# INK-USC/RE-Net

Hardware: AMD Instinct MI355X
Metric: RGCN+GRU encoder triples/s at bs=1024 n_hidden=200 (full training step, both directions) (higher is better)
Workload: dtype f32; 1 GPU; ICEWS18-shaped synthetic stream (seed 999), n_hidden=200, seq_len=10, batch=1024 per GPU, dropout=0.50, fwd+bwd both directions + clip + Adam; parallelism=dp1, global_batch=1024, nodes=99312, edges=288792

## Files before the change

re-net_amd/csrc/common.h:

```cpp
#pragma once
#include <hip/hip_runtime.h>
#include <stdint.h>
#include <stdlib.h>
#include <string.h>
#include "../../include/renet_hip.h"

#define RENET_LAUNCH(...)                         \
    do {                                          \
        (void)hipGetLastError();                  \
        hipLaunchKernelGGL(__VA_ARGS__);          \
    } while (0)

#define RENET_LAUNCH_CHECK()                      \
    do {                                          \
        hipError_t e__ = hipGetLastError();       \
        if (e__ != hipSuccess) return (int)e__;   \
    } while (0)

static inline bool renet_env_flag(const char* name, bool dflt) {
    const char* e = getenv(name);
    return (e && e[0] == '0') ? false : (e && e[0] == '1') ? true : dflt;
}
static inline int renet_env_int(const char* name, int dflt, int lo, int hi) {
    const char* e = getenv(name);
    const int v = e ? atoi(e) : dflt;
    return (v < lo || v > hi) ? dflt : v;
}
static inline bool renet_env_is(const char* name, const char* value) {
    const char* e = getenv(name);
    return e && strcmp(e, value) == 0;
}

static inline int renet_gemm_tile_order() {
    static const int v = renet_env_flag("RENET_GEMM_TILE_ORDER", true) ? renet_env_int("RENET_GEMM_PANEL_W", 8, 1, 64) : 0;
    return v;
}

static inline bool renet_dim_ok(int D) { return D == 100 || D == 200 || D == 300 || D == 400; }

__device__ __forceinline__ uint64_t renet_mix64(uint64_t x) {
    x += 0x9E3779B97F4A7C15ull;
    x = (x ^ (x >> 30)) * 0xBF58476D1CE4E5B9ull;
    x = (x ^ (x >> 27)) * 0x94D049BB133111EBull;
    return x ^ (x >> 31);
}

struct DropCfg {
    uint32_t thresh;
    float scale;
    uint64_t seed;
};

static inline DropCfg make_drop(float p, uint64_t seed) {
    DropCfg d;
    if (p <= 0.f) { d.thresh = 0; d.scale = 1.f; }
    else { d.thresh = (uint32_t)(p * 65536.f + 0.5f); d.scale = 1.f / (1.f - p); }
    d.seed = seed;
// ... 35 lines not shown
```

re-net_amd/csrc/gemm_bf16s.hip:

```cpp
#include "gemm_tiles.h"

namespace {

constexpr int P3_LOADERS = 4;
constexpr int P3_THREADS = 64 * (4 + P3_LOADERS);

struct Bf16sArgs {
    const __bf16* A;
    const __bf16* B;
    int lda, ldb;
    SplitArgs out;
};

constexpr int B1_SUB = 2;
constexpr int B1_BK = 32 * B1_SUB;
constexpr int B1_STAGE = 2 * B1_SUB * 8192;
constexpr int B1_SLOTS = 3;
constexpr size_t B1_LDS = (size_t)B1_STAGE * B1_SLOTS;
constexpr size_t B1_LDS_TALL = (size_t)B1_SUB * (256 * 64 + 8192) * B1_SLOTS;

template <bool A_TR, bool B_TR, bool TALL>
__global__ __launch_bounds__(TALL ? 768 : P3_THREADS) void gemm_bf16s_kernel(Bf16sArgs pa) {
    constexpr int TBM = TALL ? 256 : 128;
    constexpr int MW = TALL ? 8 : 4;
// ... 141 lines not shown
#pragma unroll
            for (int slab = 0; slab < 2; ++slab)
#pragma unroll
                for (int t = 0; t < 2; ++t) {
                    const char* ia = st + sb * AIMG;
                    const char* ib = st + B1_SUB * AIMG + sb * 8192;
                    if constexpr (!A_TR) fa[sb][slab][t] = *reinterpret_cast<const bf16x8*>(ia + offA[t][slab]);
                    else fa[sb][slab][t] = frag_tr(ia, offA[t], slab);
                    if constexpr (!B_TR) fb[sb][slab][t] = *reinterpret_cast<const bf16x8*>(ib + offB[t][slab]);
                    else fb[sb][slab][t] = frag_tr(ib, offB[t], slab);
                }
#pragma unroll
        for (int sb = 0; sb < B1_SUB; ++sb)
#pragma unroll
            for (int slab = 0; slab < 2; ++slab)
#pragma unroll
                for (int i = 0; i < 2; ++i)
#pragma unroll
                    for (int j = 0; j < 2; ++j)
                        acc[i][j] = __builtin_amdgcn_mfma_f32_32x32x16_bf16(fa[sb][slab][i], fb[sb][slab][j], acc[i][j], 0, 0, 0);
        asm volatile("s_waitcnt lgkmcnt(0)" ::: "memory");
        __builtin_amdgcn_s_barrier();
    }
    store_tile(g, m0, n0, z, wm, wn, lane, acc);
}

__global__ __launch_bounds__(256) void pack_bf16_kernel(const float* __restrict__ X, int R, int C, int ldx, int Rp,
                                                        int Cp, __bf16* __restrict__ P) {
    const size_t total = (size_t)Rp * Cp / 4;
    for (size_t i = (size_t)blockIdx.x * blockDim.x + threadIdx.x; i < total; i += (size_t)gridDim.x * blockDim.x) {
        const int row = (int)(i / (Cp / 4)), c = (int)(i % (Cp / 4)) * 4;
        float4 v = make_float4(0.f, 0.f, 0.f, 0.f);
        if (row < R) {
            const float* x = X + (size_t)row * ldx + c;
            if (c + 3 < C && ((ldx & 3) == 0) && ((reinterpret_cast<uintptr_t>(X) & 15) == 0)) {
                v = *reinterpret_cast<const float4*>(x);
            } else {
                if (c < C) v.x = x[0];
                if (c + 1 < C) v.y = x[1];
                if (c + 2 < C) v.z = x[2];
                if (c + 3 < C) v.w = x[3];
            }
        }
        const bf16x2 lo = __builtin_convertvector(f32x2{v.x, v.y}, bf16x2);
        const bf16x2 hi = __builtin_convertvector(f32x2{v.z, v.w}, bf16x2);
        *reinterpret_cast<uint2*>(P + (size_t)row * Cp + c) = pack4(lo, hi);
    }
// ... 52 lines not shown
}

int renet_gemm_bf16s(int a_tr, int b_tr, int M, int N, int K, float alpha, const void* Ap, int lda, const void* Bp,
                     int ldb, float beta, float* C, int ldc, const float* bias, int split_k, float* workspace,
                     size_t workspace_bytes, void* stream) {
    if (M < 0 || N < 0 || K < 1 || ldc < N || !Ap || !Bp) return RENET_ERR_BADARG;
    if (M == 0 || N == 0) return RENET_OK;
    const int Mp = (M + 255) & ~255, Np = (N + 255) & ~255, Kp = (K + 255) & ~255;
    if (lda < (a_tr ? Mp : Kp) || ldb < (b_tr ? Np : Kp) || (lda & 7) || (ldb & 7)) return RENET_ERR_BADARG;
    if (split_k < 1) split_k = 1;
    const int st_total = (K + B1_BK - 1) / B1_BK;
    if (split_k > st_total) split_k = max(st_total, 1);
    if (split_k > 1 && workspace_bytes < renet_gemm_workspace(M, N, split_k)) return RENET_ERR_WORKSPACE;
    Bf16sArgs pa;
    pa.A = (const __bf16*)Ap; pa.B = (const __bf16*)Bp;
    pa.lda = lda; pa.ldb = ldb;
    SplitArgs& g = pa.out;
    g.A = nullptr; g.B = nullptr; g.C = C; g.bias = bias; g.M = M; g.N = N; g.K = K;
    g.lda = 0; g.ldb = 0; g.ldc = ldc; g.alpha = alpha; g.beta = beta;
    g.split_k = split_k;
    g.k_tiles_per_split = max(1, (st_total + split_k - 1) / split_k);
    g.partial = workspace;
    g.xcd_order = renet_gemm_tile_order();
    hipStream_t st = (hipStream_t)stream;
    const int nbx = (N + BN - 1) / BN;
    const bool tall = (size_t)nbx * (Mp / 256) * split_k >= 256;
    dim3 grid(nbx, tall ? Mp / 256 : (M + BM - 1) / BM, split_k);
    int e;
    if (tall) {
        if (!a_tr && !b_tr) e = launch_bf16s<false, false, true>(pa, grid, st);
        else if (!a_tr && b_tr) e = launch_bf16s<false, true, true>(pa, grid, st);
        else if (a_tr && !b_tr) e = launch_bf16s<true, false, true>(pa, grid, st);
        else e = launch_bf16s<true, true, true>(pa, grid, st);
    } else {
        if (!a_tr && !b_tr) e = launch_bf16s<false, false, false>(pa, grid, st);
        else if (!a_tr && b_tr) e = launch_bf16s<false, true, false>(pa, grid, st);
        else if (a_tr && !b_tr) e = launch_bf16s<true, false, false>(pa, grid, st);
        else e = launch_bf16s<true, true, false>(pa, grid, st);
    }
    if (e != RENET_OK) return e;
    if (split_k > 1) return renet_split_reduce(workspace, split_k, M, N, alpha, beta, bias, C, ldc, st);
    return RENET_OK;
}

}
```

re-net_amd/csrc/gemm_h3.hip:

```cpp
#include <type_traits>
#include "gemm_tiles.h"
#include "gemm_skinny.h"

namespace {

typedef _Float16 f16x8 __attribute__((ext_vector_type(8)));
typedef _Float16 f16x2 __attribute__((ext_vector_type(2)));

struct H3Args {
    SplitArgs g;
    const float* maxA;
    const float* maxB;
    int nA, nB;
};

__device__ __forceinline__ float h3_scale_of(float bound, float& inv) {
    const uint32_t E = (__float_as_uint(bound) >> 23) & 0xffu;
    int f = 268 - (int)E;
    f = f > 253 ? 253 : (f < 1 ? 1 : f);
    inv = __uint_as_float((uint32_t)(254 - f) << 23);
    return __uint_as_float((uint32_t)f << 23);
}

__device__ __forceinline__ float h3_wave_max(const float* __restrict__ part, int n, int lane) {
// ... 118 lines not shown
        else store_items_h<B_CK, false, NT, BN, NIB>(sB, g.N, g.K, n0, kt * BK, tid, rb, sc_b);
        TRACE_T(wave, kt - kt0, 1);
        __syncthreads();
        TRACE_T(wave, kt - kt0, 2);
        const int k0n = min(kt + 1, kt1 - 1) * BK;
        mfma_tile_ld_h<PLANE_A, PLANE_B, NIA + NIB>(sA, sB, arow, brow, ksel, accm, accc, [&](auto ic) {
            constexpr int i = ic.value;
            if constexpr (i < NIA) la.load_item(i, k0n, ra[i]);
            else lb.load_item(i - NIA, k0n, rb[i - NIA]);
        });
        TRACE_T(wave, kt - kt0, 3);
    }
    const float inv = inv_a * inv_b;
    const bool inv_ok = inv > 0.f && inv < __uint_as_float(0x7f000000u);
#pragma unroll
    for (int i = 0; i < 2; ++i)
#pragma unroll
        for (int j = 0; j < 2; ++j)
#pragma unroll
            for (int r = 0; r < 16; ++r) {
                const float v = fmaf(accc[i][j][r], 0.00048828125f, accm[i][j][r]);
                accm[i][j][r] = inv_ok ? v * inv : (v * inv_a) * inv_b;
            }
    store_tile(g, m0, n0, z, wm, wn, lane, accm);
}

__device__ __forceinline__ float max4(float m, const float4& v) {
    return fmaxf(fmaxf(m, fmaxf(fabsf(v.x), fabsf(v.y))), fmaxf(fabsf(v.z), fabsf(v.w)));
}

template <bool FLAT>
__global__ __launch_bounds__(256) void maxabs_partials_kernel(const float* __restrict__ x, int rows, int cols, size_t ld,
                                                              float* __restrict__ part) {
    __shared__ float red[4];
    float m = 0.f;
    if constexpr (FLAT) {
        const size_t n4 = (size_t)rows * cols / 4;
        const float4* __restrict__ p = reinterpret_cast<const float4*>(x);
        const size_t stride = (size_t)gridDim.x * 256;
        size_t i = (size_t)blockIdx.x * 256 + threadIdx.x;
        float m1 = 0.f, m2 = 0.f, m3 = 0.f;
        for (; i + 3 * stride < n4; i += 4 * stride) {
            const float4 v0 = p[i], v1 = p[i + stride], v2 = p[i + 2 * stride], v3 = p[i + 3 * stride];
            m = max4(m, v0); m1 = max4(m1, v1); m2 = max4(m2, v2); m3 = max4(m3, v3);
        }
        for (; i < n4; i += stride) m = max4(m, p[i]);
        m = fmaxf(fmaxf(m, m1), fmaxf(m2, m3));
// ... 90 lines not shown

int renet_gemm_f32_h3(int ta, int tb, int M, int N, int K, float alpha, const float* A, int lda, const float* B,
                      int ldb, float beta, float* C, int ldc, const float* bias, int split_k, float* workspace,
                      size_t workspace_bytes, const float* maxA, int nA, const float* maxB, int nB, void* stream) {
    if (M < 0 || N < 0 || K < 1 || lda <= 0 || ldb <= 0 || ldc < N) return RENET_ERR_BADARG;
    if (!maxA || !maxB || nA < 1 || nB < 1 || nA > 1024 || nB > 1024) return RENET_ERR_BADARG;
    if (M == 0 || N == 0) return RENET_OK;
    const bool small_ok = (size_t)(ta ? K : M) * lda < ((size_t)1 << 30) && (size_t)(tb ? N : K) * ldb < ((size_t)1 << 30);
    if (!small_ok || ((split_k <= 1) && renet_gemm_skinny_enabled() && renet_gemm_skinny_eligible(ta, M, N, K, A, lda, B, ldb, tb)))
        return renet_gemm_f32_split(ta, tb, M, N, K, alpha, A, lda, B, ldb, beta, C, ldc, bias, split_k, workspace,
                                    workspace_bytes, stream);
    if (split_k < 1) split_k = 1;
    const int kt_total = (K + BK - 1) / BK;
    if (split_k > kt_total) split_k = max(kt_total, 1);
    if (split_k > 1 && workspace_bytes < renet_gemm_workspace(M, N, split_k)) return RENET_ERR_WORKSPACE;
    H3Args h;
    SplitArgs& g = h.g;
    g.A = A; g.B = B; g.C = C; g.bias = bias; g.M = M; g.N = N; g.K = K;
    g.lda = lda; g.ldb = ldb; g.ldc = ldc; g.alpha = alpha; g.beta = beta;
    g.split_k = split_k;
    g.k_tiles_per_split = max(1, (kt_total + split_k - 1) / split_k);
    g.partial = workspace;
    g.xcd_order = renet_gemm_tile_order();
    h.maxA = maxA; h.maxB = maxB; h.nA = nA; h.nB = nB;
    hipStream_t st = (hipStream_t)stream;
    const int nbx = (N + BN - 1) / BN;
#define RENET_H3_LAUNCH(TALLV, THR)                                                                    \
    do {                                                                                               \
        if (!ta && !tb) RENET_LAUNCH((gemm_h3_kernel<false, false, TALLV>), grid, dim3(THR), 0, st, h); \
        else if (!ta && tb) RENET_LAUNCH((gemm_h3_kernel<false, true, TALLV>), grid, dim3(THR), 0, st, h); \
        else if (ta && !tb) RENET_LAUNCH((gemm_h3_kernel<true, false, TALLV>), grid, dim3(THR), 0, st, h); \
        else RENET_LAUNCH((gemm_h3_kernel<true, true, TALLV>), grid, dim3(THR), 0, st, h);              \
    } while (0)
    if (use_tall_h3(ta, M, nbx, split_k)) {
        dim3 grid(nbx, (M + 255) / 256, split_k);
        g.xcd_order = panel_width(g.xcd_order, nbx, (int)grid.y, 256, K, split_k, 32);
        RENET_H3_LAUNCH(true, 512);
    } else {
        dim3 grid(nbx, (M + BM - 1) / BM, split_k);
        g.xcd_order = panel_width(g.xcd_order, nbx, (int)grid.y, BM, K, split_k, 64);
        RENET_H3_LAUNCH(false, 256);
    }
#undef RENET_H3_LAUNCH
    RENET_LAUNCH_CHECK();
    if (split_k > 1) return renet_split_reduce(workspace, split_k, M, N, alpha, beta, bias, C, ldc, st);
    return RENET_OK;
// ... 4 lines not shown
```

re-net_amd/csrc/gemm_planes.hip:

```cpp

#include <type_traits>
#include "gemm_tiles.h"

namespace {

struct P6Args {
    const __bf16* A;
    const __bf16* B;
    size_t a_plane, b_plane;
    int tca, tcb;
    int nbx, nby, nbz;
    const float* alpha_dev;
    float* col_out;
    SplitArgs out;
};

template <int WM>
struct P6Cfg {
    static constexpr int NW = 2 * WM;
    static constexpr int THREADS = 64 * NW;
    static constexpr int APIECES = 2 * WM;
    static constexpr int AIMG = APIECES * 1024;
    static constexpr int BIMG = 4 * 1024;
    static constexpr int PP = APIECES + 4;
// ... 2 lines not shown
    static constexpr int SLOTS = WM == 4 ? 4 : 3;
    static constexpr size_t LDS = (size_t)STAGE * SLOTS;
    static constexpr int NPIECE = 3 * PP;
    static constexpr int PER = (NPIECE + NW - 1) / NW;
    static constexpr bool UNEVEN = (NPIECE % NW) != 0;
};

__device__ __forceinline__ void p6_tile_of_index(int L, int nbx, int nby, int nbz, int xcd_order, int& bx, int& by, int& bz) {
    const int nb = nbx * nby;
    if (!xcd_order) { bz = L / nb; const int r = L - bz * nb; by = r / nbx; bx = r - by * nbx; return; }
    const int total = nb * nbz, per = total >> 3;
    const int v = L < 8 * per ? (L & 7) * per + (L >> 3) : L;
    bz = v / nb;
    const int t = v - bz * nb;
    const int ns = min(nbx, nby), nl = max(nbx, nby);
    const int w = min(ns, xcd_order);
    const int p = t / (w * nl), r = t - p * (w * nl);
    const int wp = min(w, ns - p * w);
    const int l = r / wp, sh = p * w + (r - l * wp);
    if (nby <= nbx) { bx = l; by = sh; }
    else { by = l; bx = sh; }
}

__device__ __forceinline__ void p6_store_tile(const P6Args& pa, int m0, int n0, int z, int wm, int wn, int lane,
                                              const f32x16 (&acc)[2][2]) {
    const SplitArgs& g = pa.out;
    const bool split = g.split_k > 1;
    const int half = lane >> 5;
    const int n_main = pa.col_out ? g.N - 1 : g.N;
    const bool accumulate = !split && g.beta != 0.f;
    const float alpha = pa.alpha_dev ? g.alpha * pa.alpha_dev[0] : g.alpha;
#pragma unroll
    for (int i = 0; i < 2; ++i)
#pragma unroll
        for (int j = 0; j < 2; ++j) {
            const int col = n0 + wn * 64 + j * 32 + (lane & 31);
            if (col >= g.N) continue;
            const int row_base = m0 + wm * 64 + i * 32 + 4 * half;
            float* base;
            size_t rs;
            float bv = 0.f;
            if (split) { base = g.partial + (size_t)z * g.M * g.N + col; rs = (size_t)g.N; }
            else if (col < n_main) { base = g.C + col; rs = (size_t)g.ldc; bv = g.bias ? g.bias[col] : 0.f; }
            else { base = pa.col_out; rs = 1; }
            float old[16];
#pragma unroll
            for (int r = 0; r < 16; ++r) old[r] = 0.f;
            if (accumulate) {
#pragma unroll
                for (int r = 0; r < 16; ++r) {
                    const int row = min(row_base + (r & 3) + 8 * (r >> 2), g.M - 1);
                    old[r] = base[(size_t)row * rs];
                }
            }
// ... 140 lines not shown
    auto stage_body = [&](const P6Frags& Fcur, P6Frags& Fnext, int next_slot, auto parc, bool do_issue, char* dbase) {
#ifndef RENET_P6_NOREAD
        read_frags(Fnext, next_slot, parc);
#endif
        __builtin_amdgcn_sched_barrier(0);
        static_for<0, 6>([&](auto qc) {
            constexpr int q = decltype(qc)::value;
#ifndef RENET_P6_NOMFMA
            mfma_group(Fcur, qc);
#endif
            __builtin_amdgcn_sched_barrier(0);
            if (do_issue) {
                if constexpr (WM == 4) {
                    if (five) { if constexpr (q < 5) issue_piece(dbase, std::integral_constant<int, q>{}); }
                    else { if constexpr (q >= 2) issue_piece(dbase, std::integral_constant<int, q - 2>{}); }
                } else {
                    issue_piece(dbase, std::integral_constant<int, q>{});
                }
            }
            __builtin_amdgcn_sched_barrier(0);
        });
    };

    P6Frags F0, F1;
    bool have_tile = false;
    int pm0 = 0, pn0 = 0, pz = 0;
    for (int item = blockIdx.x; item < n_items; item += gridDim.x) {
        if (have_tile) {
            p6_store_tile(pa, pm0, pn0, pz, wm, wn, lane, acc);
#pragma unroll
            for (int i = 0; i < 2; ++i)
#pragma unroll
                for (int j = 0; j < 2; ++j)
#pragma unroll
                    for (int r = 0; r < 16; ++r) acc[i][j][r] = 0.f;
        }
        int bx, by;
        p6_tile_of_index(item, pa.nbx, pa.nby, pa.nbz, g.xcd_order, bx, by, z);
        m0 = by * (64 * WM); n0 = bx * BN;
        s0 = z * g.k_tiles_per_split;
        nh = max(min(hs_total, s0 + g.k_tiles_per_split) - s0, 0);
        have_tile = true; pm0 = m0; pn0 = n0; pz = z;
        if (nh == 0) continue;
        setup_tile();
        const int npre = min(nh, NS);
        for (int j = 0; j < npre; ++j) issue(j);
        wait_left(max(npre - 2, 0));
        __builtin_amdgcn_s_barrier();
        read_frags(F0, 0, std::integral_constant<int, 0>{});
        __builtin_amdgcn_s_waitcnt(0xC07F);
        __builtin_amdgcn_s_barrier();
        int slot = 0;
        auto iter = [&](int j, auto pc) {
            constexpr int P = decltype(pc)::value;
#ifdef RENET_P6_NODMA
            const bool do_issue = j + NS < nh && j < 1;
#else
            const bool do_issue = j + NS < nh;
#endif
            char* dbase = ring6 + slot * P6_STAGE;
            slot = slot + 1 == NS ? 0 : slot + 1;
            if constexpr (P == 0) stage_body(F0, F1, slot, std::integral_constant<int, 1>{}, do_issue, dbase);
            else stage_body(F1, F0, slot, std::integral_constant<int, 0>{}, do_issue, dbase);
            wait_left(max(min(nh - 1, j + NS) - (j + 2), 0));
            __builtin_amdgcn_s_waitcnt(0xC07F);
            __builtin_amdgcn_s_barrier();
        };
        int j = 0;
        for (; j + 1 < nh; j += 2) {
            iter(j, std::integral_constant<int, 0>{});
            iter(j + 1, std::integral_constant<int, 1>{});
        }
        if (j < nh) iter(j, std::integral_constant<int, 0>{});
    }
    if (have_tile) p6_store_tile(pa, pm0, pn0, pz, wm, wn, lane, acc);
}

__global__ __launch_bounds__(256) void p6_reduce_kernel(const float* __restrict__ partial, int split_k, int M, int N,
                                                        float alpha, const float* __restrict__ alpha_dev, float beta,
                                                        const float* __restrict__ bias, float* __restrict__ C, int ldc,
                                                        float* __restrict__ col_out) {
    const size_t total = (size_t)M * N;
    const int n_main = col_out ? N - 1 : N;
    const float a = alpha_dev ? alpha * alpha_dev[0] : alpha;
    for (size_t i = (size_t)blockIdx.x * blockDim.x + threadIdx.x; i < total; i += (size_t)gridDim.x * blockDim.x) {
        const int m = (int)(i / N), n = (int)(i % N);
        float s = 0.f;
        for (int zz = 0; zz < split_k; ++zz) s += partial[(size_t)zz * total + i];
        float* p = n < n_main ? C + (size_t)m * ldc + n : col_out + m;
        float v = a * s + ((bias && n < n_main) ? bias[n] : 0.f);
        if (beta != 0.f) v += beta * (*p);
        *p = v;
    }
}

__global__ __launch_bounds__(256) void pack_planes_kernel(const float* __restrict__ X, int R, int C, int ldx, int Rp,
                                                          int Cp, int ones_col, __bf16* __restrict__ P, size_t plane) {
    const int nbc = Cp >> 6;
// ... 73 lines not shown
                      const float* bias, float* col_out, int split_k, float* workspace, size_t workspace_bytes,
                      void* stream) {
    const int n_main = col_out ? N - 1 : N;
    if (M < 0 || N < 0 || n_main < 0 || K < 1 || ldc < n_main || !Ap || !Bp) return RENET_ERR_BADARG;
    if (M == 0 || N == 0) return RENET_OK;
    const int Mp = (M + 255) & ~255, Np = (N + 127) & ~127, Kp = (K + 15) & ~15;
    if (lda < (a_tr ? Mp : Kp) || ldb < (b_tr ? Np : Kp) || (lda & 15) || (ldb & 15)) return RENET_ERR_BADARG;
    if (a_plane < (size_t)(a_tr ? Kp : Mp) * lda || b_plane < (size_t)(b_tr ? Kp : Np) * ldb) return RENET_ERR_BADARG;
    if (split_k < 1) split_k = 1;
    const int st_total = (K + 15) / 16;
    if (split_k > st_total) split_k = max(st_total, 1);
    if (split_k > 1 && workspace_bytes < renet_gemm_workspace(M, N, split_k)) return RENET_ERR_WORKSPACE;
    P6Args pa;
    pa.A = (const __bf16*)Ap; pa.B = (const __bf16*)Bp;
    pa.a_plane = a_plane; pa.b_plane = b_plane;
    pa.tca = lda >> 4; pa.tcb = ldb >> 4;
    pa.alpha_dev = alpha_dev; pa.col_out = col_out;
    SplitArgs& g = pa.out;
    g.A = nullptr; g.B = nullptr; g.C = C; g.bias = bias; g.M = M; g.N = N; g.K = K;
    g.lda = 0; g.ldb = 0; g.ldc = ldc; g.alpha = alpha; g.beta = beta;
    g.split_k = split_k;
    g.k_tiles_per_split = (max(1, (st_total + split_k - 1) / split_k) + 1) & ~1;
    g.partial = workspace;
    hipStream_t st = (hipStream_t)stream;
    static const int tile_h = renet_env_int("RENET_P6_TILE", 128, 256, 256);
    const int nbx = (N + BN - 1) / BN, nby = (M + tile_h - 1) / tile_h;
    g.xcd_order = panel_width(renet_gemm_tile_order(), nbx, nby, tile_h, K, split_k, tile_h == 256 ? 32 : 64);
    pa.nbx = nbx; pa.nby = nby; pa.nbz = split_k;
    static const bool persistent = renet_env_flag("RENET_P6_PERSISTENT", false);
    const long items = (long)nbx * nby * split_k;
    const long slots = tile_h == 256 ? 256 : 512;
    if (items > 0x7fffffffL) return RENET_ERR_UNSUPPORTED;
    dim3 grid((unsigned)((persistent && items > slots) ? slots : items), 1, 1);
    int e;
#define RENET_P6_LAUNCH(WMV)                                                   \
    do {                                                                       \
        if (!a_tr && !b_tr) e = launch_p6<false, false, WMV>(pa, grid, st);    \
        else if (!a_tr && b_tr) e = launch_p6<false, true, WMV>(pa, grid, st); \
        else if (a_tr && !b_tr) e = launch_p6<true, false, WMV>(pa, grid, st); \
        else e = launch_p6<true, true, WMV>(pa, grid, st);                     \
    } while (0)
    if (tile_h == 256) RENET_P6_LAUNCH(4);
    else RENET_P6_LAUNCH(2);
#undef RENET_P6_LAUNCH
    if (e != RENET_OK) return e;
    if (split_k > 1) {
// ... 11 lines not shown
```

re-net_amd/csrc/gemm_split.hip:

```cpp
#include <cstdlib>
#include <type_traits>
#include "gemm_tiles.h"
#include "gemm_skinny.h"

namespace {

constexpr int PLANE = BM * LDS_ROW;
constexpr int THREADS = 256;

template <bool CONTIG_K, int NT = 256, int ROWS = 128, int NI = 4>
struct ItemLoader {
    const float* base[NI];
    int kk[NI];
    size_t ld;
    int K;

    __device__ __forceinline__ void init(const float* P, int ld_, int rows, int K_, int row0, int tid) {
        ld = (size_t)ld_;
        K = K_;
#pragma unroll
        for (int i = 0; i < NI; ++i) {
            int row, k;
            item_pos<CONTIG_K, ROWS>(tid + NT * i, row, k);
            row = min(row0 + row, rows - 1);
// ... 179 lines not shown

    TRACE_V(wave, TRACE_STEPS - 1, 0, __builtin_amdgcn_s_getreg((31 << 11) | 4));
    TRACE_V(wave, TRACE_STEPS - 1, 1, __builtin_amdgcn_s_getreg((31 << 11) | 20));
    for (int kt = kt0; kt < kt1; ++kt) {
        __syncthreads();
        TRACE_T(wave, kt - kt0, 0);
        const bool k_edge = (kt + 1) * BK > g.K;
        if (a_edge || k_edge) store_items<A_CK, true, THREADS, BM, 4, RAW>(sA, g.M, g.K, m0, kt * BK, tid, ra);
        else store_items<A_CK, false, THREADS, BM, 4, RAW>(sA, g.M, g.K, m0, kt * BK, tid, ra);
        if (b_edge || k_edge) store_items<B_CK, true, THREADS, BN, 4, RAW>(sB, g.N, g.K, n0, kt * BK, tid, rb);
        else store_items<B_CK, false, THREADS, BN, 4, RAW>(sB, g.N, g.K, n0, kt * BK, tid, rb);
        TRACE_T(wave, kt - kt0, 1);
        __syncthreads();
        TRACE_T(wave, kt - kt0, 2);
        const int k0n = min(kt + 1, kt1 - 1) * BK;
        mfma_tile_ld<PL, PL, 8>(sA, sB, arow, brow, ksel, acc, [&](auto ic) {
            constexpr int i = ic.value;
            if constexpr (i < 4) la.load_item(i, k0n, ra[i]);
            else lb.load_item(i - 4, k0n, rb[i - 4]);
        });
        TRACE_T(wave, kt - kt0, 3);
    }

    store_tile(g, m0, n0, z, wm, wn, lane, acc);
}

constexpr int BMT = 256, THREADS_T = 512;
constexpr int PLANE_T = BMT * LDS_ROW;
constexpr size_t TALL_LDS = (size_t)(3 * PLANE_T + 3 * PLANE) * sizeof(__bf16);

template <bool TA, bool TB, bool RAW>
__global__ __launch_bounds__(THREADS_T) void gemm_split_tall_kernel(SplitArgs g) {
    extern __shared__ __attribute__((aligned(16))) __bf16 smem_t[];
    __bf16* sA = smem_t;
    __bf16* sB = smem_t + 3 * PLANE_T;
    const int tid = threadIdx.x;
    const int lane = tid & 63, wave = tid >> 6;
    const int wm = wave >> 1, wn = wave & 1;
    int bx, by, z;
    tile_of_block(gridDim.x, gridDim.y, g.xcd_order, bx, by, z);
    const int m0 = by * BMT, n0 = bx * BN;
    const int kt0 = z * g.k_tiles_per_split;
    const int kt_total = (g.K + BK - 1) / BK;
    const int kt1 = min(kt_total, kt0 + g.k_tiles_per_split);
    constexpr bool A_CK = !TA;
    constexpr bool B_CK = TB;
    constexpr int NIA = BMT * 8 / THREADS_T, NIB = BN * 8 / THREADS_T;
// ... 14 lines not shown
    if (kt0 < kt1) {
        la.load(kt0 * BK, ra);
        lb.load(kt0 * BK, rb);
    }
    const bool a_edge = m0 + BMT > g.M, b_edge = n0 + BN > g.N;
    const int arow = (wm * 64 + (lane & 31)) * LDS_ROW;
    const int brow = (wn * 64 + (lane & 31)) * LDS_ROW;
    const int ksel = (lane >> 5) * 8;
    for (int kt = kt0; kt < kt1; ++kt) {
        __syncthreads();
        const bool k_edge = (kt + 1) * BK > g.K;
        if (a_edge || k_edge) store_items<A_CK, true, THREADS_T, BMT, NIA, RAW>(sA, g.M, g.K, m0, kt * BK, tid, ra);
        else store_items<A_CK, false, THREADS_T, BMT, NIA, RAW>(sA, g.M, g.K, m0, kt * BK, tid, ra);
        if (b_edge || k_edge) store_items<B_CK, true, THREADS_T, BN, NIB, RAW>(sB, g.N, g.K, n0, kt * BK, tid, rb);
        else store_items<B_CK, false, THREADS_T, BN, NIB, RAW>(sB, g.N, g.K, n0, kt * BK, tid, rb);
        __syncthreads();
        const int k0n = min(kt + 1, kt1 - 1) * BK;
        mfma_tile_ld<PLANE_T, PLANE, NIA + NIB>(sA, sB, arow, brow, ksel, acc, [&](auto ic) {
            constexpr int i = ic.value;
            if constexpr (i < NIA) la.load_item(i, k0n, ra[i]);
            else lb.load_item(i - NIA, k0n, rb[i - NIA]);
        });
    }
    store_tile(g, m0, n0, z, wm, wn, lane, acc);
}

template <bool CONTIG_K>
struct TileLoader {
    const float* P;
    int off[4];
    int rowc[4], kk[4];
    int ld, K;

    __device__ __forceinline__ void init(const float* P_, int ld_, int rows, int K_, int row0, int tid) {
        P = P_; ld = ld_; K = K_;
#pragma unroll
        for (int i = 0; i < 4; ++i) {
            int row, k;
            item_pos<CONTIG_K>(tid + THREADS * i, row, k);
            row = min(row0 + row, rows - 1);
            rowc[i] = row;
            kk[i] = k;
            off[i] = CONTIG_K ? row * ld + k : row + k * ld;
        }
    }

    template <bool FAST>
// ... 187 lines not shown
        __syncthreads();
        auto step = [&](int kt, auto with_old, auto with_conv, auto fast) {
            const int cur = (kt - kt0) & 1;
            const int k0_tile = (kt + 1) * BK;
            const int k0_next = min(kt + 2, kt1 - 1) * BK;
            fused_step<TA, TB, with_old.value, with_conv.value, fast.value>(
                c, acc, smem + cur * BUF, smem + (cur ^ 1) * BUF, k0_tile, k0_next);
            __syncthreads();
        };
        using T = std::true_type;
        using F = std::false_type;
        if (kt0 + 1 < kt1) {
            step(kt0, F{}, T{}, F{});
            int kt = kt0 + 1;
            if (!c.a_edge && !c.b_edge)
                for (; kt < kt1 - 1 && (min(kt + 2, kt1 - 1) + 1) * BK <= g.K; ++kt) step(kt, T{}, T{}, T{});
            for (; kt < kt1 - 1; ++kt) step(kt, T{}, T{}, F{});
            step(kt1 - 1, T{}, F{}, F{});
        } else {
            step(kt0, F{}, F{}, F{});
        }
        static_for<0, 24>([&](auto w) { mfma_w<w.value>(c.F1, acc); });
    }
    store_tile(g, m0, n0, z, wm, wn, lane, acc);
}

template <bool CONTIG_K, bool EDGE>
__device__ __forceinline__ void store_items_1(__bf16* __restrict__ S, int rows, int K, int row0, int k0, int tid,
                                              const float4 (&r)[4]) {
#pragma unroll
    for (int i = 0; i < 4; ++i) {
        int row, k;
        item_pos<CONTIG_K>(tid + THREADS * i, row, k);
        float4 v = r[i];
        if constexpr (EDGE) v = fix_item<CONTIG_K>(v, rows, K, row0, k0, row, k);
        const f32x2 lo = {v.x, v.y}, hi = {v.z, v.w};
        *reinterpret_cast<uint2*>(S + row * LDS_ROW + k) =
            pack4(__builtin_convertvector(lo, bf16x2), __builtin_convertvector(hi, bf16x2));
    }
}

template <bool TA, bool TB>
__global__ __launch_bounds__(THREADS) void gemm_bf16_kernel(SplitArgs g) {
    __shared__ __attribute__((aligned(16))) __bf16 sA[2][PLANE];
    __shared__ __attribute__((aligned(16))) __bf16 sB[2][PLANE];
    const int tid = threadIdx.x;
    const int lane = tid & 63, wave = tid >> 6;
// ... 34 lines not shown
        if (b_edge || k_edge) store_items_1<B_CK, true>(sB[buf], g.N, g.K, n0, kt * BK, tid, rb);
        else store_items_1<B_CK, false>(sB[buf], g.N, g.K, n0, kt * BK, tid, rb);
        __syncthreads();
        if (kt + 1 < kt1) {
            la.load((kt + 1) * BK, ra);
            lb.load((kt + 1) * BK, rb);
        }
#pragma unroll
        for (int slab = 0; slab < 2; ++slab) {
            const int ko = slab * 16 + ksel;
            bf16x8 a[2], b[2];
#pragma unroll
            for (int t = 0; t < 2; ++t) {
                a[t] = *reinterpret_cast<const bf16x8*>(&sA[buf][arow + t * 32 * LDS_ROW + ko]);
                b[t] = *reinterpret_cast<const bf16x8*>(&sB[buf][brow + t * 32 * LDS_ROW + ko]);
            }
#pragma unroll
            for (int i = 0; i < 2; ++i)
#pragma unroll
                for (int j = 0; j < 2; ++j)
                    acc[i][j] = __builtin_amdgcn_mfma_f32_32x32x16_bf16(a[i], b[j], acc[i][j], 0, 0, 0);
        }
    }
    store_tile(g, m0, n0, z, wm, wn, lane, acc);
}

__global__ __launch_bounds__(256) void split_reduce_kernel(const float* __restrict__ partial, int split_k,
                                                           int M, int N, float alpha, float beta,
                                                           const float* __restrict__ bias,
                                                           float* __restrict__ C, int ldc) {
    const size_t total = (size_t)M * N;
    for (size_t i = (size_t)blockIdx.x * blockDim.x + threadIdx.x; i < total;
         i += (size_t)gridDim.x * blockDim.x) {
        const int m = (int)(i / N), n = (int)(i % N);
        float s = 0.f;
        for (int zz = 0; zz < split_k; ++zz) s += partial[(size_t)zz * total + i];
        float v = alpha * s + (bias ? bias[n] : 0.f);
        float* p = C + (size_t)m * ldc + n;
        if (beta != 0.f) v += beta * (*p);
        *p = v;
    }
}

__global__ __launch_bounds__(256) void split_reduce4_kernel(const float* __restrict__ partial, int split_k,
                                                            int M, int N, float alpha, float beta,
                                                            const float* __restrict__ bias,
                                                            float* __restrict__ C, int ldc) {
// ... 127 lines not shown
        p.kernel = 1;
        p.xcd_order = panel_width(p.xcd_order, nbx, nby, BM, K, split_k, 64);
    }
    return p;
}

static int gemm_split_launch(bool bf16_mode, int ta, int tb, int M, int N, int K, float alpha, const float* A, int lda,
                              const float* B, int ldb, float beta, float* C, int ldc, const float* bias,
                              int split_k, float* workspace, size_t workspace_bytes, void* stream) {
    if (M < 0 || N < 0 || K < 1 || lda <= 0 || ldb <= 0 || ldc < N) return RENET_ERR_BADARG;
    if (M == 0 || N == 0) return RENET_OK;
    const SplitPlan p = plan_split(bf16_mode, ta, tb, M, N, K, A, lda, B, ldb, split_k);
    split_k = p.split_k;
    const int kt_total = (K + BK - 1) / BK;
    if (split_k > 1 && workspace_bytes < renet_gemm_workspace(M, N, split_k)) return RENET_ERR_WORKSPACE;
    if (p.kernel == 3) return renet_gemm_skinny_launch(tb, M, N, K, alpha, A, lda, B, ldb, beta, C, ldc, bias, stream);
    SplitArgs g;
    g.A = A; g.B = B; g.C = C; g.bias = bias; g.M = M; g.N = N; g.K = K;
    g.lda = lda; g.ldb = ldb; g.ldc = ldc; g.alpha = alpha; g.beta = beta;
    g.split_k = split_k;
    g.k_tiles_per_split = max(1, (kt_total + split_k - 1) / split_k);
    g.partial = workspace;
    g.xcd_order = p.xcd_order;
    hipStream_t st = (hipStream_t)stream;
    const dim3 grid(p.gx, p.gy, p.gz);
    const bool raw = p.raw != 0;
    int e = RENET_OK;
    if (p.kernel == 0) {
        if (!ta && !tb) e = launch_fused<false, false>(g, grid, st);
        else if (!ta && tb) e = launch_fused<false, true>(g, grid, st);
        else if (ta && !tb) e = launch_fused<true, false>(g, grid, st);
        else e = launch_fused<true, true>(g, grid, st);
    } else if (p.kernel == 4) {
        if (!ta && !tb) RENET_LAUNCH((gemm_bf16_kernel<false, false>), grid, dim3(THREADS), 0, st, g);
        else if (!ta && tb) RENET_LAUNCH((gemm_bf16_kernel<false, true>), grid, dim3(THREADS), 0, st, g);
        else if (ta && !tb) RENET_LAUNCH((gemm_bf16_kernel<true, false>), grid, dim3(THREADS), 0, st, g);
        else RENET_LAUNCH((gemm_bf16_kernel<true, true>), grid, dim3(THREADS), 0, st, g);
    } else if (p.kernel == 2) {
#define RENET_TALL_LAUNCH(RAWV)                                                     \
        do {                                                                        \
            if (!ta && !tb) e = launch_tall<false, false, RAWV>(g, grid, st);       \
            else if (!ta && tb) e = launch_tall<false, true, RAWV>(g, grid, st);    \
            else if (ta && !tb) e = launch_tall<true, false, RAWV>(g, grid, st);    \
            else e = launch_tall<true, true, RAWV>(g, grid, st);                    \
        } while (0)
        if (raw) RENET_TALL_LAUNCH(true);
// ... 47 lines not shown
```

re-net_amd/csrc/gemm_tiles.h:

```cpp
#ifndef RENET_GEMM_TILES_H
#define RENET_GEMM_TILES_H
#include <type_traits>
#include "common.h"

__attribute__((visibility("hidden"))) int renet_split_reduce(const float* partial, int split_k, int M, int N, float alpha,
                                                             float beta, const float* bias, float* C, int ldc,
                                                             hipStream_t st);

namespace {

constexpr int BM = 128, BN = 128, BK = 32;
constexpr int LDS_ROW = 40;

typedef float f32x16 __attribute__((ext_vector_type(16)));
typedef float f32x2 __attribute__((ext_vector_type(2)));
typedef __bf16 bf16x8 __attribute__((ext_vector_type(8)));
typedef __bf16 bf16x2 __attribute__((ext_vector_type(2)));
typedef short s16x4 __attribute__((ext_vector_type(4)));

struct SplitArgs {
    const float* A;
    const float* B;
    float* C;
    const float* bias;
    int M, N, K, lda, ldb, ldc;
    float alpha, beta;
    int k_tiles_per_split;
    int split_k;
    float* partial;
    int xcd_order;
};


#ifdef RENET_GEMM_TRACE
constexpr int TRACE_BLOCKS = 64, TRACE_STEPS = 320;
__device__ unsigned long long* g_trace = nullptr;
__device__ __forceinline__ void trace_put(int wave8, int step, int slot, unsigned long long v) {
    const int flat = blockIdx.x + gridDim.x * (blockIdx.y + gridDim.y * blockIdx.z);
    if (g_trace && flat < 512 && (flat & 255) < 32 && step < TRACE_STEPS && (threadIdx.x & 63) == 0)
        g_trace[(((size_t)((flat >> 8) * 32 + (flat & 255)) * 8 + wave8) * TRACE_STEPS + step) * 4 + slot] = v;
}
#define TRACE_T(wave8, step, slot) trace_put(wave8, step, slot, __builtin_amdgcn_s_memtime())
#define TRACE_V(wave8, step, slot, v) trace_put(wave8, step, slot, (unsigned long long)(v))
#else
#define TRACE_T(wave8, step, slot)
#define TRACE_V(wave8, step, slot, v)
#endif

__device__ __forceinline__ void tile_of_block(int nbx, int nby, int xcd_order, int& bx, int& by, int& bz) {
    bz = blockIdx.z;
    if (!xcd_order) { bx = blockIdx.x; by = blockIdx.y; return; }
    const int nb = nbx * nby;
    int t;
// ... 73 lines not shown
#pragma unroll
        for (int i = 0; i < NI; ++i) load_item(i, k0, r[i]);
    }
};

__device__ __forceinline__ float4 fix_item_h(float4 v, int rows, int K, int row0, int k0, int row, int k) {
    const int kg = k0 + k;
    const bool rok = row0 + row < rows;
    if (!rok || kg >= K) v.x = 0.f;
    if (!rok || kg + 1 >= K) v.y = 0.f;
    if (!rok || kg + 2 >= K) v.z = 0.f;
    if (!rok || kg + 3 >= K) v.w = 0.f;
    return v;
}

template <int I, int N, class F>
__device__ __forceinline__ void static_for(F&& f) {
    if constexpr (I < N) {
        f(std::integral_constant<int, I>{});
        static_for<I + 1, N>(f);
    }
}

__device__ __forceinline__ void store_tile(const SplitArgs& g, int m0, int n0, int z, int wm, int wn, int lane,
                                           const f32x16 (&acc)[2][2]) {
#ifdef RENET_PROBE_NOSTORE
    if (acc[0][0][0] != 12345.678f) return;
#endif
    const bool split = g.split_k > 1;
    float* Cout = split ? g.partial + (size_t)z * g.M * g.N : g.C;
    const int ldo = split ? g.N : g.ldc;
    const int half = lane >> 5;
    const bool accumulate = !split && g.beta != 0.f;
#pragma unroll
    for (int i = 0; i < 2; ++i)
#pragma unroll
        for (int j = 0; j < 2; ++j) {
            const int col = n0 + wn * 64 + j * 32 + (lane & 31);
            if (col >= g.N) continue;
            const float bv = (!split && g.bias) ? g.bias[col] : 0.f;
            const int row_base = m0 + wm * 64 + i * 32 + 4 * half;
            float old[16];
#pragma unroll
            for (int r = 0; r < 16; ++r) old[r] = 0.f;
            if (accumulate) {
#pragma unroll
                for (int r = 0; r < 16; ++r) {
                    const int row = min(row_base + (r & 3) + 8 * (r >> 2), g.M - 1);
                    old[r] = Cout[(size_t)row * ldo + col];
                }
            }
#pragma unroll
            for (int r = 0; r < 16; ++r) {
                const int row = row_base + (r & 3) + 8 * (r >> 2);
                if (row < g.M) {
                    float* p = Cout + (size_t)row * ldo + col;
// ... 33 lines not shown
```

Before: 379,700 triples/s.

## Stage GEMM epilogue through LDS for coalesced float4 global stores

The GEMM epilogue now transposes each wave's MFMA accumulators through a per-wave LDS scratch region (reusing the operand ring or images) so that each lane writes contiguous float4 rows instead of scattered scalar column stores. This is wired into the bf16s, h3, planes and split GEMM kernels, with a block barrier before reusing operand LDS, and is on by default unless RENET_GEMM_EPILOGUE=direct. It aims to cut the uncoalesced store traffic of the epilogue. In exchange it adds LDS round-trips, extra barriers, and edge-case handling for partial tiles and the col_out column.

```diff
diff --git a/re-net_amd/csrc/common.h b/re-net_amd/csrc/common.h
--- a/re-net_amd/csrc/common.h
+++ b/re-net_amd/csrc/common.h
@@ -33,6 +33,11 @@
 
 static inline int renet_gemm_tile_order() {
     static const int v = renet_env_flag("RENET_GEMM_TILE_ORDER", true) ? renet_env_int("RENET_GEMM_PANEL_W", 8, 1, 64) : 0;
+    return v;
+}
+
+static inline int renet_gemm_epilogue_staged() {
+    static const int v = renet_env_is("RENET_GEMM_EPILOGUE", "direct") ? 0 : 1;
     return v;
 }
 
diff --git a/re-net_amd/csrc/gemm_bf16s.hip b/re-net_amd/csrc/gemm_bf16s.hip
--- a/re-net_amd/csrc/gemm_bf16s.hip
+++ b/re-net_amd/csrc/gemm_bf16s.hip
@@ -187,7 +187,8 @@
         asm volatile("s_waitcnt lgkmcnt(0)" ::: "memory");
         __builtin_amdgcn_s_barrier();
     }
-    store_tile(g, m0, n0, z, wm, wn, lane, acc);
+    static_assert((size_t)MW * EPI_WAVE_FLOATS * sizeof(float) <= (TALL ? B1_LDS_TALL : B1_LDS), "staging fits the ring");
+    store_tile(g, m0, n0, z, wm, wn, lane, acc, reinterpret_cast<float*>(ring1) + wave * EPI_WAVE_FLOATS);
 }
 
 __global__ __launch_bounds__(256) void pack_bf16_kernel(const float* __restrict__ X, int R, int C, int ldx, int Rp,
@@ -286,6 +287,7 @@
     g.k_tiles_per_split = max(1, (st_total + split_k - 1) / split_k);
     g.partial = workspace;
     g.xcd_order = renet_gemm_tile_order();
+    g.staged = renet_gemm_epilogue_staged();
     hipStream_t st = (hipStream_t)stream;
     const int nbx = (N + BN - 1) / BN;
     const bool tall = (size_t)nbx * (Mp / 256) * split_k >= 256;
diff --git a/re-net_amd/csrc/gemm_h3.hip b/re-net_amd/csrc/gemm_h3.hip
--- a/re-net_amd/csrc/gemm_h3.hip
+++ b/re-net_amd/csrc/gemm_h3.hip
@@ -164,7 +164,16 @@
                 const float v = fmaf(accc[i][j][r], 0.00048828125f, accm[i][j][r]);
                 accm[i][j][r] = inv_ok ? v * inv : (v * inv_a) * inv_b;
             }
-    store_tile(g, m0, n0, z, wm, wn, lane, accm);
+    if (tile_staged(g, z)) __syncthreads();
+    if constexpr (TALL) {
+        static_assert(8 * (EPI_WAVE_FLOATS / 2) * sizeof(float) <= 2 * PLANE_A * sizeof(_Float16), "staging fits the A image");
+        store_tile<16>(g, m0, n0, z, wm, wn, lane, accm, reinterpret_cast<float*>(sA) + __builtin_amdgcn_readfirstlane(wave) * (EPI_WAVE_FLOATS / 2));
+    } else {
+        static_assert(2 * EPI_WAVE_FLOATS * sizeof(float) <= 2 * PLANE_B * sizeof(_Float16), "staging fits an operand image");
+        const int ws = __builtin_amdgcn_readfirstlane(wave);
+        store_tile<32>(g, m0, n0, z, wm, wn, lane, accm,
+                       reinterpret_cast<float*>(ws < 2 ? sA : sB) + (ws & 1) * EPI_WAVE_FLOATS);
+    }
 }
 
 __device__ __forceinline__ float max4(float m, const float4& v) {
@@ -301,6 +310,7 @@
     g.k_tiles_per_split = max(1, (kt_total + split_k - 1) / split_k);
     g.partial = workspace;
     g.xcd_order = renet_gemm_tile_order();
+    g.staged = renet_gemm_epilogue_staged();
     h.maxA = maxA; h.maxB = maxB; h.nA = nA; h.nB = nB;
     hipStream_t st = (hipStream_t)stream;
     const int nbx = (N + BN - 1) / BN;
diff --git a/re-net_amd/csrc/gemm_planes.hip b/re-net_amd/csrc/gemm_planes.hip
--- a/re-net_amd/csrc/gemm_planes.hip
+++ b/re-net_amd/csrc/gemm_planes.hip
@@ -48,14 +48,30 @@
     else { by = l; bx = sh; }
 }
 
+__device__ __forceinline__ bool p6_staged(const P6Args& pa) {
+    const SplitArgs& g = pa.out;
+    return g.split_k > 1 ? epi_staged_ok(g, g.partial, (size_t)g.N) : epi_staged_ok(g, g.C, (size_t)g.ldc);
+}
+
 __device__ __forceinline__ void p6_store_tile(const P6Args& pa, int m0, int n0, int z, int wm, int wn, int lane,
-                                              const f32x16 (&acc)[2][2]) {
+                                              const f32x16 (&acc)[2][2], float* stage) {
+#ifdef RENET_P6_NOSTORE
+    if (acc[0][0][0] != 12345.678f) return;
+#endif
     const SplitArgs& g = pa.out;
     const bool split = g.split_k > 1;
     const int half = lane >> 5;
     const int n_main = pa.col_out ? g.N - 1 : g.N;
     const bool accumulate = !split && g.beta != 0.f;
     const float alpha = pa.alpha_dev ? g.alpha * pa.alpha_dev[0] : g.alpha;
+    if (p6_staged(pa)) {
+        EpiOut o;
+        o.M = g.M; o.bias = g.bias; o.alpha = alpha; o.beta = g.beta; o.raw = split; o.accumulate = accumulate;
+        if (split) { o.base = g.partial + (size_t)z * g.M * g.N; o.ld = (size_t)g.N; o.n_main = g.N; o.col_out = nullptr; }
+        else { o.base = g.C; o.ld = (size_t)g.ldc; o.n_main = n_main; o.col_out = pa.col_out; }
+        store_tile_staged<32>(o, stage, m0 + wm * 64, n0 + wn * 64, lane, acc);
+        return;
+    }
 #pragma unroll
     for (int i = 0; i < 2; ++i)
 #pragma unroll
@@ -242,12 +258,18 @@
         });
     };
 
+    float* stage = reinterpret_cast<float*>(ring6) + wave * EPI_WAVE_FLOATS;
+    static_assert((size_t)Cfg::NW * EPI_WAVE_FLOATS * sizeof(float) <= Cfg::LDS, "staging fits the ring");
     P6Frags F0, F1;
     bool have_tile = false;
     int pm0 = 0, pn0 = 0, pz = 0;
     for (int item = blockIdx.x; item < n_items; item += gridDim.x) {
         if (have_tile) {
-            p6_store_tile(pa, pm0, pn0, pz, wm, wn, lane, acc);
+            p6_store_tile(pa, pm0, pn0, pz, wm, wn, lane, acc, stage);
+            if (p6_staged(pa)) {
+                __builtin_amdgcn_s_waitcnt(0xC07F);
+                __builtin_amdgcn_s_barrier();
+            }
 #pragma unroll
             for (int i = 0; i < 2; ++i)
 #pragma unroll
@@ -293,7 +315,7 @@
         }
         if (j < nh) iter(j, std::integral_constant<int, 0>{});
     }
-    if (have_tile) p6_store_tile(pa, pm0, pn0, pz, wm, wn, lane, acc);
+    if (have_tile) p6_store_tile(pa, pm0, pn0, pz, wm, wn, lane, acc, stage);
 }
 
 __global__ __launch_bounds__(256) void p6_reduce_kernel(const float* __restrict__ partial, int split_k, int M, int N,
@@ -413,6 +435,7 @@
     g.split_k = split_k;
     g.k_tiles_per_split = (max(1, (st_total + split_k - 1) / split_k) + 1) & ~1;
     g.partial = workspace;
+    g.staged = renet_gemm_epilogue_staged();
     hipStream_t st = (hipStream_t)stream;
     static const int tile_h = renet_env_int("RENET_P6_TILE", 128, 256, 256);
     const int nbx = (N + BN - 1) / BN, nby = (M + tile_h - 1) / tile_h;
diff --git a/re-net_amd/csrc/gemm_split.hip b/re-net_amd/csrc/gemm_split.hip
--- a/re-net_amd/csrc/gemm_split.hip
+++ b/re-net_amd/csrc/gemm_split.hip
@@ -225,7 +225,10 @@
         TRACE_T(wave, kt - kt0, 3);
     }
 
-    store_tile(g, m0, n0, z, wm, wn, lane, acc);
+    if (tile_staged(g, z)) __syncthreads();
+    static_assert(2 * EPI_WAVE_FLOATS * sizeof(float) <= 3 * PL * sizeof(__bf16), "staging fits an operand image");
+    const int ws = __builtin_amdgcn_readfirstlane(wave);
+    store_tile(g, m0, n0, z, wm, wn, lane, acc, reinterpret_cast<float*>(ws < 2 ? sA : sB) + (ws & 1) * EPI_WAVE_FLOATS);
 }
 
 constexpr int BMT = 256, THREADS_T = 512;
@@ -286,7 +289,9 @@
             else lb.load_item(i - NIA, k0n, rb[i - NIA]);
         });
     }
-    store_tile(g, m0, n0, z, wm, wn, lane, acc);
+    if (tile_staged(g, z)) __syncthreads();
+    static_assert((THREADS_T / 64) * EPI_WAVE_FLOATS * sizeof(float) <= TALL_LDS, "staging fits the images");
+    store_tile(g, m0, n0, z, wm, wn, lane, acc, reinterpret_cast<float*>(smem_t) + __builtin_amdgcn_readfirstlane(wave) * EPI_WAVE_FLOATS);
 }
 
 template <bool CONTIG_K>
@@ -520,7 +525,7 @@
         }
         static_for<0, 24>([&](auto w) { mfma_w<w.value>(c.F1, acc); });
     }
-    store_tile(g, m0, n0, z, wm, wn, lane, acc);
+    store_tile<32, false>(g, m0, n0, z, wm, wn, lane, acc, nullptr);
 }
 
 template <bool CONTIG_K, bool EDGE>
@@ -601,7 +606,7 @@
                     acc[i][j] = __builtin_amdgcn_mfma_f32_32x32x16_bf16(a[i], b[j], acc[i][j], 0, 0, 0);
         }
     }
-    store_tile(g, m0, n0, z, wm, wn, lane, acc);
+    store_tile<32, false>(g, m0, n0, z, wm, wn, lane, acc, nullptr);
 }
 
 __global__ __launch_bounds__(256) void split_reduce_kernel(const float* __restrict__ partial, int split_k,
@@ -775,6 +780,7 @@
     g.k_tiles_per_split = max(1, (kt_total + split_k - 1) / split_k);
     g.partial = workspace;
     g.xcd_order = p.xcd_order;
+    g.staged = renet_gemm_epilogue_staged();
     hipStream_t st = (hipStream_t)stream;
     const dim3 grid(p.gx, p.gy, p.gz);
     const bool raw = p.raw != 0;
diff --git a/re-net_amd/csrc/gemm_tiles.h b/re-net_amd/csrc/gemm_tiles.h
--- a/re-net_amd/csrc/gemm_tiles.h
+++ b/re-net_amd/csrc/gemm_tiles.h
@@ -14,6 +14,7 @@
 
 typedef float f32x16 __attribute__((ext_vector_type(16)));
 typedef float f32x2 __attribute__((ext_vector_type(2)));
+typedef float f32x4 __attribute__((ext_vector_type(4)));
 typedef __bf16 bf16x8 __attribute__((ext_vector_type(8)));
 typedef __bf16 bf16x2 __attribute__((ext_vector_type(2)));
 typedef short s16x4 __attribute__((ext_vector_type(4)));
@@ -29,6 +30,7 @@
     int split_k;
     float* partial;
     int xcd_order;
+    int staged;
 };
 
 
@@ -148,8 +150,124 @@
     }
 }
 
+constexpr int EPI_PITCH = 64;
+constexpr int EPI_WAVE_FLOATS = 32 * EPI_PITCH;
+
+struct EpiOut {
+    float* base;
+    size_t ld;
+    int M, n_main;
+    float* col_out;
+    const float* bias;
+    float alpha, beta;
+    bool raw;
+    bool accumulate;
+};
+
+__device__ __forceinline__ bool epi_staged_ok(const SplitArgs& g, const float* base, size_t ld) {
+    return g.staged && ((reinterpret_cast<uintptr_t>(base) & 15) == 0) && ((ld & 3) == 0);
+}
+
+__device__ __forceinline__ bool tile_staged(const SplitArgs& g, int z) {
+    const bool split = g.split_k > 1;
+    return epi_staged_ok(g, split ? g.partial + (size_t)z * g.M * g.N : g.C, (size_t)(split ? g.N : g.ldc));
+}
+
+template <int ROWS, bool EDGE>
+__device__ __forceinline__ void store_block_staged(const EpiOut& o, float* stage, int row0, int col0, int lane,
+                                                   const f32x16 (&acc)[2][2]) {
+    typedef __attribute__((address_space(3))) float lds_f32;
+    typedef __attribute__((address_space(3))) f32x4 lds_f32x4;
+    constexpr int NK = ROWS / 4;
+    lds_f32* st = (lds_f32*)stage;
+    const int half = lane >> 5;
+    const int rl = lane >> 4;
+    const int c4 = col0 + 4 * (lane & 15);
+    const int nv = EDGE ? o.n_main - c4 : 4;
+    const bool full = nv >= 4;
+    const int cv = (EDGE && o.col_out && nv >= 0 && nv < 4) ? nv : -1;
+    float bv[4];
+#pragma unroll
+    for (int e = 0; e < 4; ++e) bv[e] = (!o.raw && o.bias && e < nv) ? o.bias[c4 + e] : 0.f;
+    auto edge_ptr = [&](int row, int e) -> float* {
+        return e < nv ? o.base + (size_t)row * o.ld + c4 + e : e == cv ? o.col_out + row : nullptr;
+    };
+#pragma unroll
+    for (int p = 0; p < 64 / ROWS; ++p) {
+        constexpr int RPB = 32 / ROWS;
+        const int i = p / RPB, r0 = (p % RPB) * (ROWS / 2);
+#pragma unroll
+        for (int j = 0; j < 2; ++j)
+#pragma unroll
+            for (int r = 0; r < ROWS / 2; ++r)
+                st[((r & 3) + 8 * (r >> 2) + 4 * half) * EPI_PITCH + j * 32 + (lane & 31)] = acc[i][j][r0 + r];
+        __builtin_amdgcn_fence(__ATOMIC_RELEASE, "wavefront");
+        __builtin_amdgcn_wave_barrier();
+        __builtin_amdgcn_fence(__ATOMIC_ACQUIRE, "wavefront");
+        f32x4 v[NK];
+#pragma unroll
+        for (int k = 0; k < NK; ++k) v[k] = *(const lds_f32x4*)(st + (rl + 4 * k) * EPI_PITCH + 4 * (lane & 15));
+        __builtin_amdgcn_s_waitcnt(0xC07F);
+        __builtin_amdgcn_fence(__ATOMIC_RELEASE, "wavefront");
+        __builtin_amdgcn_wave_barrier();
+        const int rowp = row0 + p * ROWS + rl;
+        f32x4 old[NK];
+#pragma unroll
+        for (int k = 0; k < NK; ++k) old[k] = f32x4{0.f, 0.f, 0.f, 0.f};
+        if (o.accumulate) {
+#pragma unroll
+            for (int k = 0; k < NK; ++k) {
+                const int row = rowp + 4 * k;
+                if (EDGE && row >= o.M) continue;
+                if (full) {
+                    old[k] = *reinterpret_cast<const f32x4*>(o.base + (size_t)row * o.ld + c4);
+                } else {
+#pragma unroll
+                    for (int e = 0; e < 4; ++e) {
+                        const float* q = edge_ptr(row, e);
+                        if (q) old[k][e] = *q;
+                    }
+                }
+            }
+        }
+#pragma unroll
+        for (int k = 0; k < NK; ++k) {
+            const int row = rowp + 4 * k;
+            if (EDGE && row >= o.M) continue;
+            f32x4 w;
+            if (o.raw) {
+                w = v[k];
+            } else {
+#pragma unroll
+                for (int e = 0; e < 4; ++e) w[e] = o.alpha * v[k][e] + bv[e] + (o.accumulate ? o.beta * old[k][e] : 0.f);
+            }
+            if (full) {
+                *reinterpret_cast<f32x4*>(o.base + (size_t)row * o.ld + c4) = w;
+            } else {
+#pragma unroll
+                for (int e = 0; e < 4; ++e) {
+                    float* q = edge_ptr(row, e);
+                    if (q) *q = w[e];
+                }
+            }
+        }
+    }
+}
+
+template <int ROWS>
+__device__ __forceinline__ void store_tile_staged(const EpiOut& o, float* stage, int row0, int col0, int lane,
+                                                  const f32x16 (&acc)[2][2]) {
+    static_assert(ROWS == 32 || ROWS == 16, "a pass is one or one half of a 32-row MFMA block");
+    const int n_all = o.n_main + (o.col_out ? 1 : 0);
+    if (row0 >= o.M || col0 >= n_all) return;
+    asm volatile("" : "+v"(lane));
+    if (row0 + 64 <= o.M && col0 + 64 <= o.n_main) store_block_staged<ROWS, false>(o, stage, row0, col0, lane, acc);
+    else store_block_staged<ROWS, true>(o, stage, row0, col0, lane, acc);
+}
+
+template <int ROWS = 32, bool STAGED = true>
 __device__ __forceinline__ void store_tile(const SplitArgs& g, int m0, int n0, int z, int wm, int wn, int lane,
-                                           const f32x16 (&acc)[2][2]) {
+                                           const f32x16 (&acc)[2][2], float* stage) {
 #ifdef RENET_PROBE_NOSTORE
     if (acc[0][0][0] != 12345.678f) return;
 #endif
@@ -158,6 +276,13 @@
     const int ldo = split ? g.N : g.ldc;
     const int half = lane >> 5;
     const bool accumulate = !split && g.beta != 0.f;
+    if (STAGED && epi_staged_ok(g, Cout, (size_t)ldo)) {
+        EpiOut o;
+        o.base = Cout; o.ld = (size_t)ldo; o.M = g.M; o.n_main = g.N; o.col_out = nullptr;
+        o.bias = g.bias; o.alpha = g.alpha; o.beta = g.beta; o.raw = split; o.accumulate = accumulate;
+        store_tile_staged<ROWS>(o, stage, m0 + wm * 64, n0 + wn * 64, lane, acc);
+        return;
+    }
 #pragma unroll
     for (int i = 0; i < 2; ++i)
 #pragma unroll
```

Measured after the change: 392,300 triples/s (median of 6 runs). +3.3%, better.
